# Benjamin-Lee/circkit

Hardware: NVIDIA B200
Metric: canonicalize+uniq records/sec (higher is better)
Workload: dtype u8

## Files before the change

circkit_b200/csrc/ck_lane4.cuh:

```cuda
#pragma once
#include "ck_seg2.cuh"

namespace ck {

#define CK_L4_WARPS 8u
#define CK_L4_WARP_BYTES (CK_S3_STAGE + 1024u + 384u)

__host__ __device__ __forceinline__ u64 p4_byte(u64 off, u64 rec) { return 32 * ((off >> 5) + 8 * rec); }
__host__ __device__ __forceinline__ u32 p4_strand_bytes(u32 n) { return 32u * (((n + 135u) >> 6) + 1u); }
__host__ __device__ __forceinline__ u64 p4_bytes_total(u64 total, u64 n_records) { return 32 * ((total >> 5) + 8 * n_records + 10); }

__device__ __forceinline__ u32 l4_codes4(u32 x, u32 mask, u32 &bad)
{
    const u32 idx = (x >> 1) & 0x07070707u;
    const u32 sel = __byte_perm(idx | (idx >> 4), 0, 0x4420);
    const u32 codes = __byte_perm(0x03050201u, 0x04000f0fu, sel);
    const u32 back = __byte_perm(0x47544341u, 0x4e2d0000u, sel);
    bad |= (back ^ x) & mask;
    const u32 r = __byte_perm(codes, 0, 0x0123);
    return __byte_perm(r | (r >> 4), 0, 0x4420);
}
__device__ __forceinline__ u32 l4_comp8(u32 x)
{
    const u32 m4 = x & ~(x >> 1) & 0x11111111u, m1 = (x >> 1) & ~(x >> 2) & 0x11111111u;
    return x ^ ((m4 << 2) | m1);
}
__device__ __forceinline__ u32 l4_nibrev(u32 x)
{
    const u32 r = __byte_perm(x, 0, 0x0123);
    return ((r & 0x0f0f0f0fu) << 4) | ((r >> 4) & 0x0f0f0f0fu);
}
__device__ __forceinline__ u32 l4_win(const u32 *X, u32 q)
{
    const u32 k = q >> 3;
    return __funnelshift_l(X[k + 1], X[k], 4u * (q & 7u));
}
__device__ __forceinline__ void l4_close(u32 *X, u32 n, u32 NU)
{
    const u32 v = n - 8u * (NU - 1u), f0 = X[0], f1 = X[1];
    if (v < 8u) {
        const u32 s = 4u * (8u - v);
        X[NU - 1u] |= f0 >> (4u * v);
        X[NU] = __funnelshift_l(f1, f0, s);
        X[NU + 1u] = __funnelshift_l(X[2], f1, s);
    } else { X[NU] = f0; X[NU + 1u] = f1; }
}

#define CK_P4_UNITS 260u
__global__ void __launch_bounds__(256) k_pack4(const u8 *bytes, const u64 *offsets, const u32 *lens, u8 *lane_bits, u32 n_records, u8 *p4)
{
    __shared__ u32 sh[16][2][CK_P4_UNITS];
    const u32 lane = lane_id(), hl = lane & 15u, half = lane >> 4;
    const u32 hmask = half ? 0xffff0000u : 0x0000ffffu;
    u32 *F = sh[threadIdx.x >> 4][0], *R = sh[threadIdx.x >> 4][1];
    const u32 gw = (blockIdx.x * blockDim.x + threadIdx.x) >> 5, nw = (gridDim.x * blockDim.x) >> 5;
    u32 nx_i = 2u * gw + half;
    bool nx_act = nx_i < n_records && lane_bits[nx_i] == 4;
    u64 nx_off = nx_act ? offsets[nx_i] : 0;
    u32 nx_n = nx_act ? (lens ? lens[nx_i] : (u32)(offsets[nx_i + 1] - nx_off)) : 0u;
    for (u32 i0 = 2u * gw; i0 < n_records; i0 += 2u * nw) {
        const u32 i = nx_i;
        const u64 off = nx_off;
        const u32 n = nx_n;
        bool act = nx_act && n >= 129u && n <= 2048u;
        nx_i = i0 + 2u * nw + half;
        nx_act = nx_i < n_records && lane_bits[nx_i] == 4;
        nx_off = nx_act ? offsets[nx_i] : 0;
        nx_n = nx_act ? (lens ? lens[nx_i] : (u32)(offsets[nx_i + 1] - nx_off)) : 0u;
        if (nx_act && 128u * hl < nx_n + 127u && nx_n <= 2048u) prefetch_l2(bytes + (nx_off & ~127ull) + 128u * hl);
        const u32 NU = (n + 7u) >> 3;
        const u32 *w = reinterpret_cast<const u32 *>(bytes + (off & ~3ull));
        const u32 sh8 = 8u * (u32)(off & 3u);
        u32 bad = 0;
        for (u32 j = hl; j < (act ? NU + 2u : 0u); j += 16) {
            u32 u = 0;
            if (j < NU) {
                const u32 w0 = __ldg(w + 2 * j), w1 = __ldg(w + 2 * j + 1), w2 = __ldg(w + 2 * j + 2);
                const u32 x0 = __funnelshift_r(w0, w1, sh8), x1 = __funnelshift_r(w1, w2, sh8);
                const u32 v = min(8u, n - 8u * j);
                const u32 m0 = v >= 4u ? 0xffffffffu : ~(0xffffffffu << (8u * v));
                const u32 m1 = v >= 8u ? 0xffffffffu : v > 4u ? ~(0xffffffffu << (8u * (v - 4u))) : 0u;
                u = (l4_codes4(x0, m0, bad) << 16) | l4_codes4(x1, m1, bad);
                if (v < 8u) u &= ~(0xffffffffu >> (4u * v));
            }
            F[j] = u;
        }
        __syncwarp();
        if (__ballot_sync(CK_FULL, bad != 0) & hmask) act = false;
        if (act && hl == 0) l4_close(F, n, NU);
// ... 279 lines not shown
```

circkit_b200/csrc/ck_lib.cu:

```cuda
#include <algorithm>
#include <cstdio>
#include <cstdlib>
#include <cstring>
#include <mutex>
#include <new>
#include <string>
#include <vector>

#include <cub/device/device_radix_sort.cuh>
#include <cub/device/device_scan.cuh>
#include <cub/device/device_select.cuh>
#include <cub/iterator/counting_input_iterator.cuh>

#include "../../include/circkit_b200.h"
#include "ck_kernels.cuh"
#include "ck_warp2.cuh"
#include "ck_lane2.cuh"
#include "ck_stream2.cuh"
#include "ck_stream3.cuh"
#include "ck_seg2.cuh"
#include "ck_lane4.cuh"
#include "ck_synth.cuh"
#include "ck_monomerize.cuh"
#include "ck_fasta.cuh"
// ... 185 lines not shown
    }
    return CK_OK;
}
void free_scratch(ExecScratch &s)
{
    for (int c = 0; c < CLS_COUNT; c++) {
        if (s.tie[c]) cudaFree(s.tie[c]);
        if (s.side_stream[c]) cudaStreamDestroy(s.side_stream[c]);
        if (s.ev_join[c]) cudaEventDestroy(s.ev_join[c]);
        s.tie[c] = nullptr; s.side_stream[c] = nullptr; s.ev_join[c] = nullptr;
    }
    if (s.ev_fork) cudaEventDestroy(s.ev_fork);
    if (s.seg) cudaFree(s.seg);
    if (s.huge_x) cudaFree(s.huge_x);
    if (s.huge_tie) cudaFree(s.huge_tie);
    s.huge_x = s.huge_tie = nullptr; s.huge_x_words = s.huge_tie_words = 0;
    s.ev_fork = nullptr; s.seg = nullptr;
}

template <typename K> int set_smem(ck_ctx *ctx, K kernel, u32 bytes)
{
    if (bytes > 48 * 1024) CK_CUDA(ctx, cudaFuncSetAttribute(kernel, cudaFuncAttributeMaxDynamicSharedMemorySize, (int)bytes));
    return CK_OK;
}
void s2_launch(ck_ctx *ctx, cudaStream_t st, const CanonArgs &a, int v)
{
    if (ctx->lane_kernel != 2 && a.p2_dbl) {
        const u32 g3 = 2u * (u32)ctx->num_sms, th3 = 32u * CK_S3_WARPS, sm3 = CK_S3_WARPS * CK_S3_WARP_BYTES;
#define CK_S3(V) k_canon_s3<V><<<g3, th3, sm3, st>>>(a)
        switch (v) {
        case 0: CK_S3(0); break; case 1: CK_S3(1); break; case 2: CK_S3(2); break; case 3: CK_S3(3); break;
        case 4: CK_S3(4); break; case 5: CK_S3(5); break; case 6: CK_S3(6); break; default: CK_S3(7);
        }
#undef CK_S3
        return;
    }
    const u32 g = 2u * (u32)ctx->num_sms, th = 32u * CK_S2_WARPS, sm = CK_S2_WARPS * CK_S2_WARP_BYTES;
#define CK_S2(V) k_canon_s2<V><<<g, th, sm, st>>>(a)
    switch (v) {
    case 0: CK_S2(0); break; case 1: CK_S2(1); break; case 2: CK_S2(2); break; case 3: CK_S2(3); break;
    case 4: CK_S2(4); break; case 5: CK_S2(5); break; case 6: CK_S2(6); break; default: CK_S2(7);
    }
#undef CK_S2
}

int set_attrs(ck_ctx *ctx)
{
    if (ctx->attrs_set) return CK_OK;
    int rc;
    if ((rc = set_smem(ctx, k_canon_cta<2, false>, cls_smem_bytes(CLS_C2B)))) return rc;
    if ((rc = set_smem(ctx, k_canon_cta<4, false>, cls_smem_bytes(CLS_C4)))) return rc;
    if ((rc = set_smem(ctx, k_canon_cta<8, false>, cls_smem_bytes(CLS_C8)))) return rc;
    const u32 s2 = CK_S2_WARPS * CK_S2_WARP_BYTES;
    if ((rc = set_smem(ctx, k_canon_s2<0>, s2)) || (rc = set_smem(ctx, k_canon_s2<1>, s2)) || (rc = set_smem(ctx, k_canon_s2<2>, s2)) ||
        (rc = set_smem(ctx, k_canon_s2<3>, s2)) || (rc = set_smem(ctx, k_canon_s2<4>, s2)) || (rc = set_smem(ctx, k_canon_s2<5>, s2)) ||
        (rc = set_smem(ctx, k_canon_s2<6>, s2)) || (rc = set_smem(ctx, k_canon_s2<7>, s2))) return rc;
    const u32 s3 = CK_S3_WARPS * CK_S3_WARP_BYTES;
    if ((rc = set_smem(ctx, k_canon_s3<0>, s3)) || (rc = set_smem(ctx, k_canon_s3<1>, s3)) || (rc = set_smem(ctx, k_canon_s3<2>, s3)) ||
        (rc = set_smem(ctx, k_canon_s3<3>, s3)) || (rc = set_smem(ctx, k_canon_s3<4>, s3)) || (rc = set_smem(ctx, k_canon_s3<5>, s3)) ||
        (rc = set_smem(ctx, k_canon_s3<6>, s3)) || (rc = set_smem(ctx, k_canon_s3<7>, s3))) return rc;
    const u32 l4 = CK_L4_WARPS * CK_L4_WARP_BYTES;
    if ((rc = set_smem(ctx, k_canon_l4<0>, l4)) || (rc = set_smem(ctx, k_canon_l4<1>, l4)) || (rc = set_smem(ctx, k_canon_l4<2>, l4)) ||
        (rc = set_smem(ctx, k_canon_l4<3>, l4))) return rc;
    ctx->attrs_set = true;
    return CK_OK;
}

struct CanonIO {
    const u64 *packed2; const u8 *bytes; const u64 *offsets; const u32 *lens; const u8 *lane;
    u32 n; u32 mode;
    u32 dbl = 1;
    u64 longest = 0;
    u8 *p4 = nullptr;
    u8 *out; u32 *out_start; u8 *out_strand; u64 *out_hash;
    u32 *lists; u64 lists_bytes;
    u32 *counts;
};

u64 lists_bytes_for(u64 n) { return ((16 * (n + 4) + 24 * (n + 4) + 255) & ~255ull) + (1ull << 20); }

int run_canon(ck_ctx *ctx, cudaStream_t st, ExecScratch &scr, const CanonIO &io, u32 class_mask)
{
    if (io.n == 0) return CK_OK;
    int rc = set_attrs(ctx);
    if (rc) return rc;
    CK_CUDA(ctx, cudaMemsetAsync(io.counts, 0, 64 * sizeof(u32), st));
    int only = -1;
    if (class_mask && (class_mask & (class_mask - 1)) == 0)
        for (int c = 0; c < CLS_COUNT; c++) if (class_mask == (1u << c)) only = c;
    const u64 stride = ((u64)io.n + 4) & ~3ull;
    u32 *k0 = io.lists, *k1 = k0 + stride, *v0 = k1 + stride, *v1 = v0 + stride;
    if (io.lists_bytes < 16 * stride) return fail(ctx, CK_ERR_ARG, "sort workspace too small");
    const bool fastv = io.packed2 && !(io.mode & 1u) && (!io.out || (io.mode & 2u)) && io.out_start && io.out_strand;
    u32 window_shift = 32, top_bit = 13;
    if (fastv && only < 0) {
        window_shift = 16;
        u32 wbits = 0;
        while ((((u64)io.n - 1) >> window_shift) >> wbits) wbits++;
        top_bit = std::max(14u, 5u + wbits);
    }
    const bool l4_run = fastv && only < 0 && ctx->l4_kernel && io.p4 && io.lane && io.bytes && (!class_mask || (class_mask & (1u << CLS_W4)));
    if (l4_run) {
        cudaEvent_t e0 = nullptr, e1 = nullptr;
        if (ctx->timing) { CK_CUDA(ctx, cudaEventCreate(&e0)); CK_CUDA(ctx, cudaEventCreate(&e1)); CK_CUDA(ctx, cudaEventRecord(e0, st)); }
        k_pack4<<<std::min<u32>((io.n + 15) / 16, 16u * (u32)ctx->num_sms), 256, 0, st>>>(io.bytes, io.offsets, io.lens, const_cast<u8 *>(io.lane), io.n, io.p4);
        if (ctx->timing) { CK_CUDA(ctx, cudaEventRecord(e1, st)); ctx->ev_pairs[CLS_COUNT + 5].push_back(e0); ctx->ev_pairs[CLS_COUNT + 5].push_back(e1); }
        ctx->launches++;
    }
    const int sort_bits = (int)top_bit + 1;
    const bool lane_checks = fastv && only >= 0 && io.lane == nullptr &&
                             (only == CLS_W2S || only == CLS_W2M || only == CLS_W2L || only == CLS_W2X);
    if (!lane_checks) {
        ClassifyArgs ca{io.offsets, io.lens, io.lane, io.n, k0, v0, io.counts, only >= 0 ? (1u << only) : 0u, window_shift, top_bit};
        k_classify<<<std::min<u32>((io.n + 255) / 256, 16u * (u32)ctx->num_sms), 256, 0, st>>>(ca);
        ctx->launches++;
    }
    const u32 *sorted = nullptr;
    u32 *retry = v0;
    if (only < 0) {
        cub::DoubleBuffer<u32> keys(k0, k1), vals(v0, v1);
        void *tmp = v1 + stride;
        size_t tmp_bytes = (size_t)(io.lists_bytes - 16 * stride), need = 0;
        cub::DeviceRadixSort::SortPairs(nullptr, need, keys, vals, (int)io.n, 0, sort_bits, st);
        if (need > tmp_bytes) return fail(ctx, CK_ERR_ARG, "sort workspace too small");
        CK_CUDA(ctx, cub::DeviceRadixSort::SortPairs(tmp, need, keys, vals, (int)io.n, 0, sort_bits, st));
        sorted = vals.Current();
        retry = vals.Alternate();
        k_list_starts<<<1, 32, 0, st>>>(io.counts);
        ctx->launches += 2;
    }
    const u32 lane_classes = (1u << CLS_W2S) | (1u << CLS_W2M) | (1u << CLS_W2L) | (1u << CLS_W2X);
    auto timed = [&](int slot, cudaEvent_t &e0, cudaEvent_t &e1, bool begin, cudaStream_t on) -> cudaError_t {
        if (!ctx->timing) return cudaSuccess;
        if (begin) {
            cudaError_t e = cudaEventCreate(&e0); if (e != cudaSuccess) return e;
            e = cudaEventCreate(&e1); if (e != cudaSuccess) return e;
            return cudaEventRecord(e0, on);
        }
        ctx->ev_pairs[slot].push_back(e0); ctx->ev_pairs[slot].push_back(e1);
        return cudaEventRecord(e1, on);
    };
    auto base_args = [&](int c) {
        CanonArgs a{};
        a.packed2 = io.packed2; a.p2_dbl = io.dbl; a.bytes = io.bytes; a.offsets = io.offsets; a.lens = io.lens;
        a.max_n = cls_max_n(c); a.min_n = cls_min_n(c);
        a.out = io.out; a.out_start = io.out_start; a.out_strand = io.out_strand; a.out_hash = io.out_hash;
        a.scratch = scr.tie[c]; a.scratch_stride = kCls[c].bits ? cls_tie_words(c) : 0;
        a.smem_units = kCls[c].bits ? cls_units(c) : 0; a.xglobal = nullptr; a.mode = io.mode;
        a.retry = retry; a.retry_counts = io.counts + 32;
        return a;
    };
    const bool lane_run = fastv && (only >= 0 ? ((lane_classes >> only) & 1u) != 0 : (!class_mask || (class_mask & lane_classes)));
    if (lane_run) {
        CanonArgs a = base_args(only >= 0 ? only : CLS_W2S);
        if (only >= 0) { a.list = nullptr; a.count = nullptr; a.n_direct = io.n; }
        else { a.list = sorted; a.count = io.counts + 12; a.n_direct = 0; a.min_n = 1; a.max_n = cls_max_n(CLS_W2X); }
        const int v = (a.out_hash ? CK_W2_HASH : 0) | (a.out ? CK_W2_OUT : 0) | (a.list ? CK_W2_LIST : 0);
        a.mode |= ctx->s3_debug;
        cudaEvent_t e0 = nullptr, e1 = nullptr;
        CK_CUDA(ctx, timed(CLS_COUNT, e0, e1, true, st));
        s2_launch(ctx, st, a, v);
        CK_CUDA(ctx, timed(CLS_COUNT, e0, e1, false, st));
        ctx->launches++;
    }
    const u32 seg_classes = (1u << CLS_C2A) | (1u << CLS_C2B);
    const bool seg_run = fastv && only < 0 && ctx->seg_kernel && io.dbl && (!class_mask || (class_mask & seg_classes));
// ... 1418 lines not shown
```

circkit_b200/csrc/ck_seg2.cuh:

```cuda
#pragma once
#include "ck_stream3.cuh"

namespace ck {

#define CK_SEG_WARPS 8u
#define CK_SEG_WARP_BYTES CK_S3_STAGE
#define CK_SEG_SCRATCH_U64 (8u * 448u)

__device__ __forceinline__ u32 seg_step_min32(u32 x0, u32 x1, u32 x2)
{
    u32 m = min(x0, x1);
#pragma unroll
    for (int i = 1; i < 16; i += 2) {
        const u32 a = __funnelshift_l(x1, x0, 2 * i), b = i + 1 < 16 ? __funnelshift_l(x1, x0, 2 * i + 2) : a;
        m = min(min(m, a), b);
    }
#pragma unroll
    for (int i = 1; i < 16; i += 2) {
        const u32 a = __funnelshift_l(x2, x1, 2 * i), b = i + 1 < 16 ? __funnelshift_l(x2, x1, 2 * i + 2) : a;
        m = min(min(m, a), b);
    }
    return m;
}
__device__ __forceinline__ u32 seg_step_min32_masked(u32 x0, u32 x1, u32 x2, u32 valid)
{
    u32 m = 0xffffffffu;
#pragma unroll
    for (int i = 0; i < 16; i++) {
        const u32 a = i ? __funnelshift_l(x1, x0, 2 * i) : x0, b = i ? __funnelshift_l(x2, x1, 2 * i) : x1;
        if ((valid >> i) & 1u) m = min(m, a);
        if ((valid >> (16 + i)) & 1u) m = min(m, b);
    }
    return m;
}
__device__ __forceinline__ void seg_track(u32 &m1k, u32 &m1t, u32 &m2k, u32 k, u32 tag)
{
    const bool lt = k < m1k;
    m2k = lt ? m1k : min(m2k, k);
    m1t = lt ? tag : m1t;
    m1k = min(m1k, k);
}

template <int V>
__global__ void __launch_bounds__(32 * CK_SEG_WARPS, 2) k_canon_seg(CanonArgs a, u64 *seg_scratch)
{
    extern __shared__ __align__(16) u32 smem[];
    constexpr bool want_hash = (V & CK_W2_HASH) != 0, want_out = (V & CK_W2_OUT) != 0;
    const u32 lane = lane_id(), wid = threadIdx.x >> 5;
    const u32 aux = (u32)__cvta_generic_to_shared(smem) + wid * CK_SEG_WARP_BYTES;
    u64 *S = seg_scratch + (size_t)(blockIdx.x * CK_SEG_WARPS + wid) * CK_SEG_SCRATCH_U64;
    const u32 count = *a.count;
    a.list += a.count[16];
    const u8 *arena = reinterpret_cast<const u8 *>(a.packed2);
    const u32 st_w = aux + 128u * (lane >> 1);
    const u32 st_j = 4u * (lane & 1u) + ((lane >> 1) & 3u);
    const u32 st_w0 = st_w + 16u * (st_j & 7u), st_w1 = st_w + 16u * ((st_j + 1u) & 7u);
    const u32 st_w2 = st_w + 16u * ((st_j + 2u) & 7u), st_w3 = st_w + 16u * ((st_j + 3u) & 7u);
    const u32 st_r = aux + 128u * (lane >> 3) + 16u * (((lane & 3u) + 4u * ((lane >> 2) & 1u) + ((lane >> 3) & 3u)) & 7u);
    const u64 *sec = reinterpret_cast<const u64 *>(c_secret);

    for (;;) {
        u32 e = 0;
        if (lane == 0) e = atomicAdd(a.retry_counts + 29, 1u);
        e = __shfl_sync(CK_FULL, e, 0);
        if (e >= count) break;
        const u32 rec = a.list[e];
        const u64 off = a.offsets[rec];
        const u32 n = a.lens ? a.lens[rec] : (u32)(a.offsets[rec + 1] - off);
        const u8 *base = arena + 8ull * p2_word(off, rec, 1u);
        u8 *dst = want_out ? a.out + out_byte(off, rec) : nullptr;

        const u32 S1 = ((n + 31) >> 5) - 1;
        const u32 octs = (S1 + 4) >> 2;
        const u32 per = (octs + 31) >> 5;
        const u32 o0 = min(lane * per, octs), o1 = min(o0 + per, octs);
        u32 m1k = 0xffffffffu, m1t = 0, m2k = 0xffffffffu;
        if (o0 < o1) {
            Oct OA = ldg256_here(base + 32 * o0), OB = ldg256_here(base + 32 * (o0 + 1)), OC = ldg256_here(base + 32 * (o0 + 2));
            u32 r0 = w2_revcomp(OA.lo.x);
#pragma unroll 1
            for (u32 j = o0; j < o1; j++) {
                const Oct ON = ldg256_here(base + 32 * min(j + 3, octs + 1));
                if ((j & 1u) == 0) prefetch_l2(base + 32 * min(j + 8, octs + 1));
                const u32 r1 = w2_revcomp(OA.lo.y), r2 = w2_revcomp(OA.lo.z), r3 = w2_revcomp(OA.lo.w);
                const u32 r4 = w2_revcomp(OA.hi.x), r5 = w2_revcomp(OA.hi.y), r6 = w2_revcomp(OA.hi.z);
                const u32 r7 = w2_revcomp(OA.hi.w), r8 = w2_revcomp(OB.lo.x);
                const u32 t = 4 * j;
#define CK_SEG_STEP(tt, x0, x1, x2, q0, q1, q2)                                                                      \
                if ((tt) < S1) {                                                                                     \
// ... 218 lines not shown
```

circkit_b200/csrc/ck_stream3.cuh:

```cuda
#pragma once
#include "ck_stream2.cuh"

namespace ck {

#define CK_S3_WARPS 8u
#define CK_S3_STAGE 2048u
#define CK_S3_WARP_BYTES (CK_S3_STAGE + 1024u + 384u + 2560u)

struct Oct { uint4 lo, hi; };

__device__ __forceinline__ Oct ldg256_here(const void *p)
{
    Oct o;
    asm volatile("ld.global.nc.v8.u32 {%0, %1, %2, %3, %4, %5, %6, %7}, [%8];"
                 : "=r"(o.lo.x), "=r"(o.lo.y), "=r"(o.lo.z), "=r"(o.lo.w), "=r"(o.hi.x), "=r"(o.hi.y), "=r"(o.hi.z), "=r"(o.hi.w)
                 : "l"(p));
    return o;
}
__device__ __forceinline__ void ldg256_if(Oct &o, const void *p, u32 on)
{
    asm volatile("{\n.reg .pred q;\nsetp.ne.u32 q, %9, 0;\n@q ld.global.nc.v8.u32 {%0, %1, %2, %3, %4, %5, %6, %7}, [%8];\n}"
                 : "+r"(o.lo.x), "+r"(o.lo.y), "+r"(o.lo.z), "+r"(o.lo.w), "+r"(o.hi.x), "+r"(o.hi.y), "+r"(o.hi.z), "+r"(o.hi.w)
                 : "l"(p), "r"(on));
}

template <int V>
__global__ void __launch_bounds__(32 * CK_S3_WARPS, 2) k_canon_s3(CanonArgs a)
{
    extern __shared__ __align__(16) u32 smem[];
    constexpr bool want_hash = (V & CK_W2_HASH) != 0, want_out = (V & CK_W2_OUT) != 0, use_list = (V & CK_W2_LIST) != 0;
    const u32 lane = lane_id(), wid = threadIdx.x >> 5;
    const u32 aux = (u32)__cvta_generic_to_shared(smem) + wid * CK_S3_WARP_BYTES;
    const u32 offs = aux + CK_S3_STAGE + 16u * lane;
    const u32 recs = aux + CK_S3_STAGE + 1024u + 4u * lane;
    const u32 head = aux + CK_S3_STAGE + 1024u + 384u + 80u * lane;
    const u32 count = use_list ? *a.count : a.n_direct;
    if (use_list) a.list += a.count[16];
    const u8 *arena = reinterpret_cast<const u8 *>(a.packed2);
    const bool pf_scan = !(a.mode & 0x100u);
    auto fetch_head = [&](u64 off1, u32 n1, u32 rec1) {
        const u8 *nb = arena + 8ull * p2_word(off1, rec1, 1u);
        const u32 s1 = n1 >= 128u ? ((n1 + 31u) >> 5) - 1u : 0u;
        cp_async16(head, nb); cp_async16(head + 16, nb + 16); cp_async16(head + 32, nb + 32); cp_async16(head + 48, nb + 48);
        cp_async8(head + 64, nb + 8 * s1); cp_async8(head + 72, nb + 8 * s1 + 8);
    };
    const bool has_lens = a.lens != nullptr;
    auto fetch_offsets = [&](u32 rec, u32 slot) {
        cp_async8(offs + 512u * slot, a.offsets + rec);
        if (has_lens) cp_async4(offs + 512u * slot + 8u, a.lens + rec);
        else cp_async8(offs + 512u * slot + 8u, a.offsets + rec + 1);
    };
    auto length_of = [&](const uint4 &oe) { return has_lens ? oe.z : oe.z - oe.x; };
    auto claim = [&]() {
        u32 v = 0;
        if (lane == 0) v = atomicAdd(a.retry_counts + 28, 1u);
        return __shfl_sync(CK_FULL, v, 0) * 32u;
    };
    u32 b0 = claim(), b1 = claim(), b2 = claim();
    u32 rq = 0;
    {
        const u32 i0 = b0 + lane, i1 = b1 + lane, i2 = b2 + lane;
        u32 r0 = i0, r1 = i1;
        if (use_list) {
            r0 = i0 < count ? a.list[i0] : 0u; r1 = i1 < count ? a.list[i1] : 0u; rq = i2 < count ? a.list[i2] : 0u;
            sts32(recs, r0); sts32(recs + 128, r1);
        }
        if (i0 < count) fetch_offsets(r0, 0);
        if (i1 < count) fetch_offsets(r1, 1);
        cp_async_wait_all();
        __syncwarp();
        if (i0 < count) {
            const uint4 oe = lds128(offs);
            fetch_head(((u64)oe.y << 32) | oe.x, length_of(oe), r0);
        }
    }
    const u32 st_w = aux + 128u * (lane >> 1);
    const u32 st_j = 4u * (lane & 1u) + ((lane >> 1) & 3u);
    const u32 st_w0 = st_w + 16u * (st_j & 7u), st_w1 = st_w + 16u * ((st_j + 1u) & 7u);
    const u32 st_w2 = st_w + 16u * ((st_j + 2u) & 7u), st_w3 = st_w + 16u * ((st_j + 3u) & 7u);
    const u32 st_r = aux + 128u * (lane >> 3) + 16u * (((lane & 3u) + 4u * ((lane >> 2) & 1u) + ((lane >> 3) & 3u)) & 7u);

    u32 kb = 0;
    for (; b0 < count; kb++) {
        const u32 sl = kb & 1u;
        const u32 idx = b0 + lane;
        const bool have = idx < count;
        const u32 b3 = claim();
        cp_async_wait_all();
        __syncwarp();
        u32 rec = idx; u64 off = 0; u32 n = 0;
        {
            const uint4 oe = lds128(offs + 512u * sl);
            if (use_list) rec = lds32(recs + 128u * (kb % 3u));
            if (have) { off = ((u64)oe.y << 32) | oe.x; n = length_of(oe); } else rec = 0;
            const u32 idx2 = b2 + lane;
            if (idx2 < count) fetch_offsets(use_list ? rq : idx2, sl);
            if (use_list) {
                sts32(recs + 128u * ((kb + 2u) % 3u), rq);
                const u32 idx3 = b3 + lane;
                rq = idx3 < count ? a.list[idx3] : 0u;
            }
        }
        const uint4 H0 = lds128(head), H1 = lds128(head + 16), H2 = lds128(head + 32), H3 = lds128(head + 48), HT = lds128(head + 64);
        if (b1 + lane < count) {
            const uint4 oe = lds128(offs + 512u * (sl ^ 1u));
            const u32 rec1 = use_list ? lds32(recs + 128u * ((kb + 1u) % 3u)) : b1 + lane;
            fetch_head(((u64)oe.y << 32) | oe.x, length_of(oe), rec1);
        }
        const bool in_class = have && (use_list || (n >= a.min_n && n <= a.max_n));
        if (!use_list && have && !in_class) atomicAdd(a.retry_counts + ((int)CLS_HUGE - 32), 1u);
        bool fast = in_class && n >= (want_hash ? 129u : 128u);
        const u8 *base = arena + 8ull * p2_word(off, rec, 1u);
        u8 *dst = want_out ? a.out + out_byte(off, rec) : nullptr;
        u32 os = 0;
        u64 h = 0;
        const u32 nn = fast ? n : 128u;

        const u32 S1 = ((nn + 31) >> 5) - 1;
        const u32 S1max = __reduce_max_sync(CK_FULL, fast ? S1 : 0u);
        const u32 omax = fast ? ((S1 - 1) >> 2) + 1 : 0u;
        u32 m1 = 0xffffffffu, m2 = 0xffffffffu, m3 = 0xffffffffu;
        const bool pf_long = pf_scan && S1max >= 32u;
        const uint2 l01 = make_uint2(HT.x, HT.y);
        const u32 l2 = HT.z;
        {
            Oct OA, OB, OC;
            OA.lo = H0; OA.hi = H1; OB.lo = H2; OB.hi = H3;
            u32 r0 = w2_revcomp(OA.lo.x);
            const u32 iters = (S1max + 3) >> 2;
#ifndef CK_S3_AHEAD
#ifndef CK_S3_SCAN_UNROLL
#define CK_S3_AHEAD 3u
#else
#define CK_S3_AHEAD 2u
#endif
#endif
#define CK_S3_STEP(t, x0, x1, x2, q0, q1, q2)                                                                          \
            {                                                                                                          \
                const u32 kf = t2_key_hi(w2_step_min16(x0, x1, x2)), kr = t2_key_hi(w2_step_min16(q2, q1, q0));        \
                const u32 tag = ((t) < S1) ? 2 * (t) : 0xffff0000u;                                                    \
                t3_track2(m1, m2, m3, kf | tag, kr | (tag + 1));                                                       \
            }
#define CK_S3_SCAN(O, O1, O2)                                                                                          \
            {                                                                                                          \
                O2 = ldg256_here(base + 32 * min(j + CK_S3_AHEAD, omax));                                              \
                if ((j & 1u) == 0 && pf_long) prefetch_l2(base + 32 * min(j + 8, omax));                                          \
                const u32 r1 = w2_revcomp(O.lo.y), r2 = w2_revcomp(O.lo.z), r3 = w2_revcomp(O.lo.w);                   \
                const u32 r4 = w2_revcomp(O.hi.x), r5 = w2_revcomp(O.hi.y), r6 = w2_revcomp(O.hi.z);                   \
                const u32 r7 = w2_revcomp(O.hi.w), r8 = w2_revcomp(O1.lo.x);                                           \
                const u32 t = 4 * j;                                                                                   \
                CK_S3_STEP(t, O.lo.x, O.lo.y, O.lo.z, r0, r1, r2)                                                      \
                CK_S3_STEP(t + 1, O.lo.z, O.lo.w, O.hi.x, r2, r3, r4)                                                  \
                CK_S3_STEP(t + 2, O.hi.x, O.hi.y, O.hi.z, r4, r5, r6)                                                  \
                CK_S3_STEP(t + 3, O.hi.z, O.hi.w, O1.lo.x, r6, r7, r8)                                                 \
                r0 = r8;                                                                                               \
                if (++j >= iters) break;                                                                               \
            }
            if (iters) {
                u32 j = 0;
#ifndef CK_S3_SCAN_UNROLL
                OC = ldg256_here(base + 32 * min(2u, omax));
#if CK_S3_AHEAD == 4
                Oct OD = ldg256_here(base + 32 * min(3u, omax));
#endif
#pragma unroll 1
                for (;;) {
                    Oct ON;
                    CK_S3_SCAN(OA, OB, ON)
#if CK_S3_AHEAD == 4
                    OA = OB; OB = OC; OC = OD; OD = ON;
#else
                    OA = OB; OB = OC; OC = ON;
#endif
                }
#else
#pragma unroll 1
                for (;;) {
                    CK_S3_SCAN(OA, OB, OC)
                    CK_S3_SCAN(OB, OC, OA)
                    CK_S3_SCAN(OC, OA, OB)
                }
#endif
            }
#undef CK_S3_SCAN
#undef CK_S3_STEP
        }
        {
            const int dT = (int)nn + 7 - 32 * (int)S1;
            const int dA = dT + 9;
#define CK_T2_PAD(d) __funnelshift_rc(0xffffffffu, 0u, 2u * (u32)min(max((d), 0), 16))
            const u32 pT0 = CK_T2_PAD(dT), pT1 = CK_T2_PAD(dT - 16), pT2 = CK_T2_PAD(dT - 32);
            const u32 pA0 = CK_T2_PAD(dA), pA1 = CK_T2_PAD(dA - 16), pA2 = CK_T2_PAD(dA - 32);
#undef CK_T2_PAD
            const u32 kf = t2_key_hi(w2_step_min16(l01.x | pT0, l01.y | pT1, l2 | pT2));
            const u32 kr = t2_key_hi(w2_step_min16(w2_revcomp(l2 & ~pA2), w2_revcomp(l01.y & ~pA1), w2_revcomp(l01.x & ~pA0)));
            t3_track2(m1, m2, m3, kf | (2 * S1), kr | (2 * S1 + 1));
        }
        {
            const u32 mm1 = fast ? m1 : 0u;
            const bool eq2 = (m1 ^ m2) < 0x10000u, eq3 = (m1 ^ m3) < 0x10000u;
            const u32 hits1 = s3_replay(base, nn, mm1);
            u32 hits2 = 0;
            const bool pair = fast && eq2 && !eq3;
            if (__any_sync(CK_FULL, pair)) hits2 = s3_replay(base, nn, pair ? m2 : mm1);
            const u32 c1 = __popc(hits1), c2 = pair ? __popc(hits2) : 0u;
            u32 st = s3_start(nn, mm1, __ffs(hits1) - 1), strand = mm1 & 1u;
            if (!(c1 == 1 && !eq2)) {
                if (fast && !eq3 && c1 + c2 == 2 && (!eq2 || pair)) {
                    const u32 mb = c2 ? m2 : mm1;
                    const u32 stb = s3_start(nn, mb, c2 ? __ffs(hits2) - 1 : 31u - __clz(hits1)), sb = mb & 1u;
                    const u32 ea = s3_ext16(base, nn, strand, st), eb = s3_ext16(base, nn, sb, stb);
                    if (ea == eb) fast = false;
                    else if (eb < ea) { st = stb; strand = sb; }
                } else fast = false;
            }
            os = (st << 1) | strand;
            if (!fast) os = 0;
        }
        if (want_out || want_hash) {
            const u32 strand = os & 1u;
            const u32 T = strand ? 0x41434754u : 0x54474341u;
            const u32 sa = strand ? 0x5140u : 0x2637u, sb = strand ? 0x7362u : 0x0415u, rot = strand ? 16u : 0u;
            int p0 = strand ? (int)nn - 16 - (int)(os >> 1) : (int)(os >> 1);
            if (p0 < 0) p0 += (int)nn;
            const u32 Bv = strand ? (u32)p0 + nn - 112u : (u32)p0;
            const u32 xs = 2u * (Bv & 15u);
            const bool b2 = (Bv & 64u) != 0, b1 = (Bv & 32u) != 0, b0s = (Bv & 16u) != 0;
            const int ostep = fast ? (strand ? -32 : 32) : 0;
            const int olim = (int)(((2u * nn + 127u) >> 7) << 5);
            const u32 nchunks = fast ? (nn + 15) >> 4 : 0u;
            const u32 nfull = fast ? (nn - 1) >> 6 : 0u;
            u64 acc0 = CK_P32_3, acc1 = CK_P64_1, acc2 = CK_P64_2, acc3 = CK_P64_3;
            u64 acc4 = CK_P64_4, acc5 = CK_P32_2, acc6 = CK_P64_5, acc7 = CK_P32_1;
            const u32 nbr = (want_hash && fast && nn <= 240u) ? nn >> 4 : 0u;
            const bool any_mid = want_hash && __any_sync(CK_FULL, nbr != 0);
            u64 mida = 0, midb = 0;
            u32 og[4] = {0, 0, 0, 0}; int orem[4] = {0, 0, 0, 0};
            if (want_out) {
                const u32 gr = (u32)((dst - a.out) >> 4);
#pragma unroll
                for (u32 i = 0; i < 4; i++) {
                    og[i] = __shfl_sync(CK_FULL, gr, 8 * i + (lane >> 2)) + (lane & 3u);
                    orem[i] = (int)__shfl_sync(CK_FULL, nchunks, 8 * i + (lane >> 2)) - (int)(lane & 3u);
                }
            }
            const u64 *sec = reinterpret_cast<const u64 *>(c_secret);
            const u32 o0 = fast ? (Bv >> 7) << 5 : 0u;
            int onext = fast ? (strand ? (int)o0 - 32 : (int)o0 + 64) : 0;
            Oct R0 = ldg256_here(base + o0), R1 = ldg256_here(base + o0 + 32);
#ifdef CK_S3_OG2
            uint4 *op[4];
            _Pragma("unroll") for (u32 i = 0; i < 4; i++) op[i] = reinterpret_cast<uint4 *>(a.out) + og[i];
#define CK_S3_STORE4 _Pragma("unroll") for (u32 i = 0; i < 4; i++) { if (orem[i] > (int)(4u * s)) op[i][4u * s] = g[i]; }
#else
#define CK_S3_STORE4 _Pragma("unroll") for (u32 i = 0; i < 4; i++) { if (orem[i] > 0) reinterpret_cast<uint4 *>(a.out)[og[i]] = g[i]; og[i] += 4; orem[i] -= 4; }
#endif
#define CK_T2_SCR(A, I) do { A ^= A >> 47; A ^= sec[16 + I]; A *= CK_P32_1; } while (0)
#define CK_S3_ROUND(MID)                                                                                            \
            {                                                                                                       \
                uint4 v[4];                                                                                         \
                v[0] = t2_ascii16(__funnelshift_l(W0, W0, rot), T, sa, sb);                                         \
                v[1] = t2_ascii16(__funnelshift_l(W1, W1, rot), T, sa, sb);                                         \
                v[2] = t2_ascii16(__funnelshift_l(W2, W2, rot), T, sa, sb);                                         \
                v[3] = t2_ascii16(__funnelshift_l(W3, W3, rot), T, sa, sb);                                         \
                if (want_hash && s < nfull) {                                                                       \
                    const u32 ks = s & 15u;                                                                         \
                    t2_acc16(acc0, acc1, v[0], sec[ks + 0], sec[ks + 1]);                                           \
                    t2_acc16(acc2, acc3, v[1], sec[ks + 2], sec[ks + 3]);                                           \
                    t2_acc16(acc4, acc5, v[2], sec[ks + 4], sec[ks + 5]);                                           \
                    t2_acc16(acc6, acc7, v[3], sec[ks + 6], sec[ks + 7]);                                           \
                    if (ks == 15u) {        \
                        CK_T2_SCR(acc0, 0); CK_T2_SCR(acc1, 1); CK_T2_SCR(acc2, 2); CK_T2_SCR(acc3, 3);             \
                        CK_T2_SCR(acc4, 4); CK_T2_SCR(acc5, 5); CK_T2_SCR(acc6, 6); CK_T2_SCR(acc7, 7);             \
                    }                                                                                               \
                }                                                                                                   \
                if (MID) {                                                                                          \
                    _Pragma("unroll") for (u32 k = 0; k < 4; k++) {                                                 \
                        const u32 i = 4 * s + k;                                                                    \
                        const u64 lo = ((u64)v[k].y << 32) | v[k].x, hi = ((u64)v[k].w << 32) | v[k].z;             \
                        if (i < 8) { const u64 t = mul128_fold64(lo ^ sec[2 * i], hi ^ sec[2 * i + 1]); if (i < nbr) mida += t; }      \
                        else if (i < 15) { const u64 t = mul128_fold64(lo ^ c_midsec[2 * i - 16], hi ^ c_midsec[2 * i - 15]); if (i < nbr) midb += t; } \
                    }                                                                                               \
                }                                                                                                   \
                if (want_out) {                                                                                     \
                    sts128(st_w0, v[0]); sts128(st_w1, v[1]); sts128(st_w2, v[2]); sts128(st_w3, v[3]);             \
                    __syncwarp();                                                                                   \
                    uint4 g[4];                                                                                     \
                    _Pragma("unroll") for (u32 i = 0; i < 4; i++) g[i] = lds128(st_r + 512u * i);                   \
                    CK_S3_STORE4                                                                                    \
                    __syncwarp();                                                                                   \
                }                                                                                                   \
            }
#ifdef CK_S3_UNROLL_HH
#define CK_S3_HH_LOOP _Pragma("unroll")
#else
#define CK_S3_HH_LOOP _Pragma("unroll 1")
#endif
#define CK_S3_PAIR(LO, UP, MID)                                                                                     \
            {                                                                                                       \
                u32 w[8];                                                                                           \
                {                                                                                                   \
                                                  \
                    const u32 a0 = b2 ? LO.hi.x : LO.lo.x, a1 = b2 ? LO.hi.y : LO.lo.y, a2 = b2 ? LO.hi.z : LO.lo.z;   \
                    const u32 a3 = b2 ? LO.hi.w : LO.lo.w, a4 = b2 ? UP.lo.x : LO.hi.x, a5 = b2 ? UP.lo.y : LO.hi.y;   \
                    const u32 a6 = b2 ? UP.lo.z : LO.hi.z, a7 = b2 ? UP.lo.w : LO.hi.w, a8 = b2 ? UP.hi.x : UP.lo.x;   \
                    const u32 a9 = b2 ? UP.hi.y : UP.lo.y, a10 = b2 ? UP.hi.z : UP.lo.z, a11 = b2 ? UP.hi.w : UP.lo.w; \
                    const u32 c0 = b1 ? a2 : a0, c1 = b1 ? a3 : a1, c2 = b1 ? a4 : a2, c3 = b1 ? a5 : a3, c4 = b1 ? a6 : a4; \
                    const u32 c5 = b1 ? a7 : a5, c6 = b1 ? a8 : a6, c7 = b1 ? a9 : a7, c8 = b1 ? a10 : a8, c9 = b1 ? a11 : a9; \
                    const u32 y0 = b0s ? c1 : c0, y1 = b0s ? c2 : c1, y2 = b0s ? c3 : c2, y3 = b0s ? c4 : c3, y4 = b0s ? c5 : c4; \
                    const u32 y5 = b0s ? c6 : c5, y6 = b0s ? c7 : c6, y7 = b0s ? c8 : c7, y8 = b0s ? c9 : c8;      \
                    w[0] = __funnelshift_l(y1, y0, xs); w[1] = __funnelshift_l(y2, y1, xs);                         \
                    w[2] = __funnelshift_l(y3, y2, xs); w[3] = __funnelshift_l(y4, y3, xs);                         \
                    w[4] = __funnelshift_l(y5, y4, xs); w[5] = __funnelshift_l(y6, y5, xs);                         \
                    w[6] = __funnelshift_l(y7, y6, xs); w[7] = __funnelshift_l(y8, y7, xs);                         \
                }                                                                                                   \
                if (s + 2 < rounds) {           \
                    const u8 *ad = base + (u32)min(max(onext, 0), olim);                                            \
                    ldg256_if(LO, ad, strand ^ 1u);                                                                 \
                    ldg256_if(UP, ad, strand);                                                                      \
                    onext += ostep;                                                                                 \
                }                                                                                                   \
                CK_S3_HH_LOOP for (u32 hh = 0; hh < 2u && s < rounds; hh++, s++) {                                 \
                    u32 W0, W1, W2, W3;                                                                             \
                    if (hh == 0) { W0 = strand ? w[7] : w[0]; W1 = strand ? w[6] : w[1]; W2 = strand ? w[5] : w[2]; W3 = strand ? w[4] : w[3]; } \
                    else { W0 = strand ? w[3] : w[4]; W1 = strand ? w[2] : w[5]; W2 = strand ? w[1] : w[6]; W3 = strand ? w[0] : w[7]; } \
                    CK_S3_ROUND(MID)                                                                                \
                }                                                                                                   \
                if (s >= rounds) break;                                                                             \
            }
            const u32 rounds = __reduce_max_sync(CK_FULL, (nchunks + 3) >> 2);
            if (rounds) {
                u32 s = 0;
                if (any_mid) {
#pragma unroll 1
                    for (;;) {
                        CK_S3_PAIR(R0, R1, true)
                        CK_S3_PAIR(R1, R0, true)
                    }
                } else {
#pragma unroll 1
                    for (;;) {
                        CK_S3_PAIR(R0, R1, false)
                        CK_S3_PAIR(R1, R0, false)
                    }
                }
            }
#undef CK_S3_PAIR
#undef CK_S3_ROUND
#undef CK_S3_STORE4
            if (want_hash) {
                const u32 Bl = strand ? (u32)p0 + 16u : (u32)p0 + nn - 64u;
                const u8 *ad = base + ((Bl >> 6) << 4);
                const uint4 XA = ldg128_here(ad), XB = ldg128_here(ad + 16);
                const u32 xa = (Bl >> 4) & 3u, xl = 2u * Bl;
                const bool a2 = (xa & 2u) != 0, a1 = (xa & 1u) != 0;
                const u32 y0 = a2 ? XA.z : XA.x, y1 = a2 ? XA.w : XA.y, y2 = a2 ? XB.x : XA.z, y3 = a2 ? XB.y : XA.w;
                const u32 y4 = a2 ? XB.z : XB.x, y5 = a2 ? XB.w : XB.y;
                const u32 u0 = a1 ? y1 : y0, u1 = a1 ? y2 : y1, u2 = a1 ? y3 : y2, u3 = a1 ? y4 : y3, u4 = a1 ? y5 : y4;
                const u32 w0 = __funnelshift_l(u1, u0, xl), w1 = __funnelshift_l(u2, u1, xl);
                const u32 w2 = __funnelshift_l(u3, u2, xl), w3 = __funnelshift_l(u4, u3, xl);
                const u32 W0 = strand ? w3 : w0, W1 = strand ? w2 : w1, W2 = strand ? w1 : w2, W3 = strand ? w0 : w3;
                {
                    const uint4 v0 = t2_ascii16(__funnelshift_l(W0, W0, rot), T, sa, sb);
                    t2_acc16(acc0, acc1, v0, c_lastsec[0], c_lastsec[1]);
                    const uint4 v1 = t2_ascii16(__funnelshift_l(W1, W1, rot), T, sa, sb);
                    t2_acc16(acc2, acc3, v1, c_lastsec[2], c_lastsec[3]);
                    const uint4 v2 = t2_ascii16(__funnelshift_l(W2, W2, rot), T, sa, sb);
                    t2_acc16(acc4, acc5, v2, c_lastsec[4], c_lastsec[5]);
                    const uint4 v3 = t2_ascii16(__funnelshift_l(W3, W3, rot), T, sa, sb);
                    t2_acc16(acc6, acc7, v3, c_lastsec[6], c_lastsec[7]);
                }
                u64 r = (u64)nn * CK_P64_1;
                r += mul128_fold64(acc0 ^ c_mergesec[0], acc1 ^ c_mergesec[1]);
                r += mul128_fold64(acc2 ^ c_mergesec[2], acc3 ^ c_mergesec[3]);
                r += mul128_fold64(acc4 ^ c_mergesec[4], acc5 ^ c_mergesec[5]);
                r += mul128_fold64(acc6 ^ c_mergesec[6], acc7 ^ c_mergesec[7]);
                h = xxh3_avalanche(r);
            }
            if (any_mid) {
                const u32 q = strand ? (u32)p0 + 16u : (u32)p0 + nn - 16u;
                const u8 *ad = base + ((q >> 4) << 2);
                const u32 w = __funnelshift_l(ldg32(ad + 4), ldg32(ad), 2u * q);
                const uint4 vv = t2_ascii16(__funnelshift_l(w, w, rot), T, sa, sb);
                const u64 lo = ((u64)vv.y << 32) | vv.x, hi = ((u64)vv.w << 32) | vv.z;
                const u64 tail = mul128_fold64(lo ^ c_midsec[14], hi ^ c_midsec[15]);
                if (nbr) h = xxh3_avalanche(xxh3_avalanche((u64)nn * CK_P64_1 + mida) + midb + tail);
            }
#undef CK_T2_SCR
        }
        if (fast) {
            const u32 start = os >> 1, strand = os & 1u;
            a.out_start[rec] = strand ? (n - 1 - start) : start;
            a.out_strand[rec] = (u8)strand;
            if (want_hash) a.out_hash[rec] = h;
        } else if (in_class) {
            const int c = n <= cls_max_n(CLS_W2S) ? CLS_W2S : n <= cls_max_n(CLS_W2M) ? CLS_W2M : n <= cls_max_n(CLS_W2L) ? CLS_W2L
                        : n <= cls_max_n(CLS_W2X) ? CLS_W2X : n <= cls_max_n(CLS_C2A) ? CLS_C2A : CLS_C2B;
            const u32 k = atomicAdd(a.retry_counts + c, 1u);
            a.retry[a.retry_counts[16 + c] + k] = rec;
        }
        __syncwarp();
        b0 = b1; b1 = b2; b2 = b3;
    }
}

}
```

Measured before the change: 1.456 billion.

## Store canonical output directly with 256-bit global stores and simplify scan prefetch

Result: slower. 1.394 billion, median of 6 (-4.3%).

```diff
diff --git a/circkit_b200/csrc/ck_lane4.cuh b/circkit_b200/csrc/ck_lane4.cuh
--- a/circkit_b200/csrc/ck_lane4.cuh
+++ b/circkit_b200/csrc/ck_lane4.cuh
@@ -4,7 +4,7 @@
 namespace ck {
 
 #define CK_L4_WARPS 8u
-#define CK_L4_WARP_BYTES (CK_S3_STAGE + 1024u + 384u)
+#define CK_L4_WARP_BYTES (CK_STAGE_BYTES + 1024u + 384u)
 
 __host__ __device__ __forceinline__ u64 p4_byte(u64 off, u64 rec) { return 32 * ((off >> 5) + 8 * rec); }
 __host__ __device__ __forceinline__ u32 p4_strand_bytes(u32 n) { return 32u * (((n + 135u) >> 6) + 1u); }
diff --git a/circkit_b200/csrc/ck_lib.cu b/circkit_b200/csrc/ck_lib.cu
--- a/circkit_b200/csrc/ck_lib.cu
+++ b/circkit_b200/csrc/ck_lib.cu
@@ -291,6 +291,7 @@
 int run_canon(ck_ctx *ctx, cudaStream_t st, ExecScratch &scr, const CanonIO &io, u32 class_mask)
 {
     if (io.n == 0) return CK_OK;
+    if (io.out && (io.mode & 2u) && ((uintptr_t)io.out & 31u)) return fail(ctx, CK_ERR_ARG, "aligned output arena not 32-byte aligned");
     int rc = set_attrs(ctx);
     if (rc) return rc;
     CK_CUDA(ctx, cudaMemsetAsync(io.counts, 0, 64 * sizeof(u32), st));
diff --git a/circkit_b200/csrc/ck_seg2.cuh b/circkit_b200/csrc/ck_seg2.cuh
--- a/circkit_b200/csrc/ck_seg2.cuh
+++ b/circkit_b200/csrc/ck_seg2.cuh
@@ -4,7 +4,8 @@
 namespace ck {
 
 #define CK_SEG_WARPS 8u
-#define CK_SEG_WARP_BYTES CK_S3_STAGE
+#define CK_STAGE_BYTES 2048u
+#define CK_SEG_WARP_BYTES CK_STAGE_BYTES
 #define CK_SEG_SCRATCH_U64 (8u * 448u)
 
 __device__ __forceinline__ u32 seg_step_min32(u32 x0, u32 x1, u32 x2)
diff --git a/circkit_b200/csrc/ck_stream3.cuh b/circkit_b200/csrc/ck_stream3.cuh
--- a/circkit_b200/csrc/ck_stream3.cuh
+++ b/circkit_b200/csrc/ck_stream3.cuh
@@ -4,8 +4,7 @@
 namespace ck {
 
 #define CK_S3_WARPS 8u
-#define CK_S3_STAGE 2048u
-#define CK_S3_WARP_BYTES (CK_S3_STAGE + 1024u + 384u + 2560u)
+#define CK_S3_WARP_BYTES (1024u + 384u + 2560u)
 
 struct Oct { uint4 lo, hi; };
 
@@ -23,6 +22,11 @@
                  : "+r"(o.lo.x), "+r"(o.lo.y), "+r"(o.lo.z), "+r"(o.lo.w), "+r"(o.hi.x), "+r"(o.hi.y), "+r"(o.hi.z), "+r"(o.hi.w)
                  : "l"(p), "r"(on));
 }
+__device__ __forceinline__ void stg256(void *p, const uint4 &a, const uint4 &b)
+{
+    asm volatile("st.global.v8.u32 [%0], {%1, %2, %3, %4, %5, %6, %7, %8};"
+                 :: "l"(p), "r"(a.x), "r"(a.y), "r"(a.z), "r"(a.w), "r"(b.x), "r"(b.y), "r"(b.z), "r"(b.w) : "memory");
+}
 
 template <int V>
 __global__ void __launch_bounds__(32 * CK_S3_WARPS, 2) k_canon_s3(CanonArgs a)
@@ -31,9 +35,9 @@
     constexpr bool want_hash = (V & CK_W2_HASH) != 0, want_out = (V & CK_W2_OUT) != 0, use_list = (V & CK_W2_LIST) != 0;
     const u32 lane = lane_id(), wid = threadIdx.x >> 5;
     const u32 aux = (u32)__cvta_generic_to_shared(smem) + wid * CK_S3_WARP_BYTES;
-    const u32 offs = aux + CK_S3_STAGE + 16u * lane;
-    const u32 recs = aux + CK_S3_STAGE + 1024u + 4u * lane;
-    const u32 head = aux + CK_S3_STAGE + 1024u + 384u + 80u * lane;
+    const u32 offs = aux + 16u * lane;
+    const u32 recs = aux + 1024u + 4u * lane;
+    const u32 head = aux + 1024u + 384u + 80u * lane;
     const u32 count = use_list ? *a.count : a.n_direct;
     if (use_list) a.list += a.count[16];
     const u8 *arena = reinterpret_cast<const u8 *>(a.packed2);
@@ -74,12 +78,6 @@
             fetch_head(((u64)oe.y << 32) | oe.x, length_of(oe), r0);
         }
     }
-    const u32 st_w = aux + 128u * (lane >> 1);
-    const u32 st_j = 4u * (lane & 1u) + ((lane >> 1) & 3u);
-    const u32 st_w0 = st_w + 16u * (st_j & 7u), st_w1 = st_w + 16u * ((st_j + 1u) & 7u);
-    const u32 st_w2 = st_w + 16u * ((st_j + 2u) & 7u), st_w3 = st_w + 16u * ((st_j + 3u) & 7u);
-    const u32 st_r = aux + 128u * (lane >> 3) + 16u * (((lane & 3u) + 4u * ((lane >> 2) & 1u) + ((lane >> 3) & 3u)) & 7u);
-
     u32 kb = 0;
     for (; b0 < count; kb++) {
         const u32 sl = kb & 1u;
@@ -124,27 +122,18 @@
         const uint2 l01 = make_uint2(HT.x, HT.y);
         const u32 l2 = HT.z;
         {
-            Oct OA, OB, OC;
+            Oct OA, OB, OC, OD;
             OA.lo = H0; OA.hi = H1; OB.lo = H2; OB.hi = H3;
             u32 r0 = w2_revcomp(OA.lo.x);
             const u32 iters = (S1max + 3) >> 2;
-#ifndef CK_S3_AHEAD
-#ifndef CK_S3_SCAN_UNROLL
-#define CK_S3_AHEAD 3u
-#else
-#define CK_S3_AHEAD 2u
-#endif
-#endif
 #define CK_S3_STEP(t, x0, x1, x2, q0, q1, q2)                                                                          \
             {                                                                                                          \
                 const u32 kf = t2_key_hi(w2_step_min16(x0, x1, x2)), kr = t2_key_hi(w2_step_min16(q2, q1, q0));        \
                 const u32 tag = ((t) < S1) ? 2 * (t) : 0xffff0000u;                                                    \
                 t3_track2(m1, m2, m3, kf | tag, kr | (tag + 1));                                                       \
             }
-#define CK_S3_SCAN(O, O1, O2)                                                                                          \
+#define CK_S3_SCAN(O, O1)                                                                                              \
             {                                                                                                          \
-                O2 = ldg256_here(base + 32 * min(j + CK_S3_AHEAD, omax));                                              \
-                if ((j & 1u) == 0 && pf_long) prefetch_l2(base + 32 * min(j + 8, omax));                                          \
                 const u32 r1 = w2_revcomp(O.lo.y), r2 = w2_revcomp(O.lo.z), r3 = w2_revcomp(O.lo.w);                   \
                 const u32 r4 = w2_revcomp(O.hi.x), r5 = w2_revcomp(O.hi.y), r6 = w2_revcomp(O.hi.z);                   \
                 const u32 r7 = w2_revcomp(O.hi.w), r8 = w2_revcomp(O1.lo.x);                                           \
@@ -158,29 +147,17 @@
             }
             if (iters) {
                 u32 j = 0;
-#ifndef CK_S3_SCAN_UNROLL
                 OC = ldg256_here(base + 32 * min(2u, omax));
-#if CK_S3_AHEAD == 4
-                Oct OD = ldg256_here(base + 32 * min(3u, omax));
-#endif
+                OD = ldg256_here(base + 32 * min(3u, omax));
 #pragma unroll 1
                 for (;;) {
-                    Oct ON;
-                    CK_S3_SCAN(OA, OB, ON)
-#if CK_S3_AHEAD == 4
-                    OA = OB; OB = OC; OC = OD; OD = ON;
-#else
-                    OA = OB; OB = OC; OC = ON;
-#endif
+                    if (pf_long) prefetch_l2(base + 32 * min(j + 8, omax));
+                    CK_S3_SCAN(OA, OB)
+                    CK_S3_SCAN(OB, OC)
+                    OA = OC; OB = OD;
+                    OC = ldg256_here(base + 32 * min(j + 2, omax));
+                    OD = ldg256_here(base + 32 * min(j + 3, omax));
                 }
-#else
-#pragma unroll 1
-                for (;;) {
-                    CK_S3_SCAN(OA, OB, OC)
-                    CK_S3_SCAN(OB, OC, OA)
-                    CK_S3_SCAN(OC, OA, OB)
-                }
-#endif
             }
 #undef CK_S3_SCAN
 #undef CK_S3_STEP
@@ -235,26 +212,11 @@
             const u32 nbr = (want_hash && fast && nn <= 240u) ? nn >> 4 : 0u;
             const bool any_mid = want_hash && __any_sync(CK_FULL, nbr != 0);
             u64 mida = 0, midb = 0;
-            u32 og[4] = {0, 0, 0, 0}; int orem[4] = {0, 0, 0, 0};
-            if (want_out) {
-                const u32 gr = (u32)((dst - a.out) >> 4);
-#pragma unroll
-                for (u32 i = 0; i < 4; i++) {
-                    og[i] = __shfl_sync(CK_FULL, gr, 8 * i + (lane >> 2)) + (lane & 3u);
-                    orem[i] = (int)__shfl_sync(CK_FULL, nchunks, 8 * i + (lane >> 2)) - (int)(lane & 3u);
-                }
-            }
+            const u32 nhalves = fast ? (nn + 31) >> 5 : 0u;
             const u64 *sec = reinterpret_cast<const u64 *>(c_secret);
             const u32 o0 = fast ? (Bv >> 7) << 5 : 0u;
             int onext = fast ? (strand ? (int)o0 - 32 : (int)o0 + 64) : 0;
             Oct R0 = ldg256_here(base + o0), R1 = ldg256_here(base + o0 + 32);
-#ifdef CK_S3_OG2
-            uint4 *op[4];
-            _Pragma("unroll") for (u32 i = 0; i < 4; i++) op[i] = reinterpret_cast<uint4 *>(a.out) + og[i];
-#define CK_S3_STORE4 _Pragma("unroll") for (u32 i = 0; i < 4; i++) { if (orem[i] > (int)(4u * s)) op[i][4u * s] = g[i]; }
-#else
-#define CK_S3_STORE4 _Pragma("unroll") for (u32 i = 0; i < 4; i++) { if (orem[i] > 0) reinterpret_cast<uint4 *>(a.out)[og[i]] = g[i]; og[i] += 4; orem[i] -= 4; }
-#endif
 #define CK_T2_SCR(A, I) do { A ^= A >> 47; A ^= sec[16 + I]; A *= CK_P32_1; } while (0)
 #define CK_S3_ROUND(MID)                                                                                            \
             {                                                                                                       \
@@ -283,12 +245,8 @@
                     }                                                                                               \
                 }                                                                                                   \
                 if (want_out) {                                                                                     \
-                    sts128(st_w0, v[0]); sts128(st_w1, v[1]); sts128(st_w2, v[2]); sts128(st_w3, v[3]);             \
-                    __syncwarp();                                                                                   \
-                    uint4 g[4];                                                                                     \
-                    _Pragma("unroll") for (u32 i = 0; i < 4; i++) g[i] = lds128(st_r + 512u * i);                   \
-                    CK_S3_STORE4                                                                                    \
-                    __syncwarp();                                                                                   \
+                    if (2u * s < nhalves) stg256(dst + 64u * s, v[0], v[1]);                                        \
+                    if (2u * s + 1u < nhalves) stg256(dst + 64u * s + 32u, v[2], v[3]);                             \
                 }                                                                                                   \
             }
 #ifdef CK_S3_UNROLL_HH
@@ -347,7 +305,6 @@
             }
 #undef CK_S3_PAIR
 #undef CK_S3_ROUND
-#undef CK_S3_STORE4
             if (want_hash) {
                 const u32 Bl = strand ? (u32)p0 + 16u : (u32)p0 + nn - 64u;
                 const u8 *ad = base + ((Bl >> 6) << 4);
```
